# yoyololicon/pytorch-NMF

Hardware: AMD Instinct MI355X
Metric: MU GFLOP/s (algorithmic 8*N*C*R per iteration), dense NMF 4096x65536 rank-128 beta=1; MU iterations/s alongside (higher is better)
Workload: dtype f16; 1 GPU; NMF 4096x65536 rank=128 beta=1 (BASELINE configs[1]); preset=cfg1, rows=4096, cols_per_gpu=65536, rank=128, precision=f16, parallelism=single GPU, nsplit_h=16, nsplit_w=1, block_rows_h=256, block_rows_w=256, launch=eager launches

## Files before the change

### include/nmfmu.h

```cpp
#ifndef NMFMU_H_
#define NMFMU_H_

#include <stddef.h>
#include <stdint.h>

#ifdef __cplusplus
extern "C" {
#endif

#define NMFMU_ABI_VERSION 10

#define NMFMU_OK 0
#define NMFMU_ERR_UNSUPPORTED (-2)
#define NMFMU_ERR_ARG (-3)
#define NMFMU_ERR_ALLOC (-4)

#define NMFMU_PREC_BF16 0
#define NMFMU_PREC_BF16X3 1
#define NMFMU_PREC_F16 2
#define NMFMU_PREC_F16X 3
#define NMFMU_PREC_F16R 4

#define NMFMU_BETA_KL 0
#define NMFMU_BETA_EUC 1
#define NMFMU_BETA_IS 2
#define NMFMU_BETA_GEN 3

#define NMFMU_STAGE_REG 0
#define NMFMU_STAGE_DMA 1
#define NMFMU_STAGE_DMA_NOP2 3
#define NMFMU_STAGE_DMA_LDSTR 4
#define NMFMU_STAGE_DMA_SP128 5
#define NMFMU_STAGE_DMA_SPLIT 2

typedef struct nmfmu_factor {
  float* f;
  void* p1_hi;
  void* p1_lo;
  void* p2_hi;
  void* p2_lo;
  float* colsum;
  float* colsum_part;
  int32_t rows;
  int32_t rows_pad;
} nmfmu_factor;

typedef struct nmfmu_step {
  const void* xp;
  nmfmu_factor owner;
  nmfmu_factor panel;
  float* slab_num;
  float* slab_den;
  int32_t rank;
  int32_t r_pad;
  int32_t nsplit;
  int32_t precision;
  int32_t stage;
  int32_t block_rows;
  float beta;
  float gamma;
  float l1, l2;
  uint32_t* status;
  void* stamps;
} nmfmu_step;

// ... 334 lines not shown
```

### pytorch-nmf_amd/csrc/nmfmu_capi.hip

```cpp
#include <hip/hip_runtime.h>
#include <stdint.h>

#include <algorithm>
#include <cstdlib>
#include <new>
#include <vector>

#include "../../include/nmfmu.h"
#include "nmfmu_aux.h"
#include "nmfmu_fused.h"
#include "nmfmu_pp.h"
#include "nmfmu_sp.h"
#include "nmfmu_sp2.h"
#include "nmfmu_sp128.h"

#ifndef NMFMU_SP
#define NMFMU_SP 1
#endif
#ifndef NMFMU_SP2
#define NMFMU_SP2 1
#endif
#ifndef NMFMU_FUSE_APPLY_TWO_ACC
#define NMFMU_FUSE_APPLY_TWO_ACC 1
#endif
// ... 25 lines not shown
static bool pp_ldstr_eligible(int r_pad, int precision, float beta) {
  return pp_eligible(r_pad, precision, beta) && pp_trl_available(r_pad, is_f16(precision) ? kOpF16 : kOpBf16, kModeMU);
}
static bool sp128_eligible(int r_pad, int precision, float beta) {
  return pp_ldstr_eligible(r_pad, precision, beta) && precision == NMFMU_PREC_F16 && sp128_available(r_pad, kOpF16, kModeMU);
}
static bool sp_eligible(int r_pad, int precision, float beta) {
  return NMFMU_SP && nmfmu_beta_kind(beta) == NMFMU_BETA_KL && r_pad == 256 && precision == NMFMU_PREC_F16;
}
static bool sp2_eligible(int r_pad, int precision, float beta) {
  const int k = nmfmu_beta_kind(beta);
  return NMFMU_SP2 && (k == NMFMU_BETA_IS || k == NMFMU_BETA_GEN) && r_pad == 128 && precision == NMFMU_PREC_F16;
}
static int kernel_beta_kind(float beta) {
  if (beta == 0.5f) return kSqrt;
  if (beta == 1.5f) return kSqrt3;
  return nmfmu_beta_kind(beta);
}

struct GramRef {
  const float* gram;
  const void* hi;
  const void* lo;
  const float* scale;
};

int fused_dispatch(const nmfmu_step* st, int mode, float* loss_part, int M, int K, hipStream_t s,
                   const float* fuse_kl_den = nullptr, bool fuse_apply = false, const GramRef* gm = nullptr) {
  if (!st || !st->owner.p1_hi || !st->panel.p1_hi) return NMFMU_ERR_ARG;
  if (!st->xp && (mode == kModeMU || mode == kModeXB)) return NMFMU_ERR_ARG;
  if (st->owner.rows_pad % kRowPad || st->panel.rows_pad % kRowPad) return NMFMU_ERR_ARG;
  if (st->block_rows != 128 && st->block_rows != 256) return NMFMU_ERR_ARG;
  if (st->stage != NMFMU_STAGE_DMA && st->stage != NMFMU_STAGE_DMA_SPLIT && st->stage != NMFMU_STAGE_DMA_NOP2 &&
      st->stage != NMFMU_STAGE_DMA_LDSTR && st->stage != NMFMU_STAGE_DMA_SP128)
    return NMFMU_ERR_UNSUPPORTED;
  const bool sp128 = st->stage == NMFMU_STAGE_DMA_SP128;
  const bool ldstr = (st->stage == NMFMU_STAGE_DMA_LDSTR || sp128) && mode != kModeLoss;
  if (ldstr && (mode != kModeMU || st->block_rows != 256 || !pp_ldstr_eligible(st->r_pad, st->precision, st->beta)))
    return NMFMU_ERR_UNSUPPORTED;
  if (sp128 && !sp128_eligible(st->r_pad, st->precision, st->beta)) return NMFMU_ERR_UNSUPPORTED;
  if (st->stage == NMFMU_STAGE_DMA_SPLIT && mode == kModeMU && !(st->precision == NMFMU_PREC_BF16X3)) {
    if (nmfmu_beta_kind(st->beta) != NMFMU_BETA_KL || st->block_rows != 128) return NMFMU_ERR_UNSUPPORTED;
    mode = kModeMU2;
  }
  if (st->r_pad != pad_rank(st->rank) || st->nsplit < 1) return NMFMU_ERR_ARG;
  const bool x3 = st->precision == NMFMU_PREC_BF16X3;
  if (x3 && (!st->owner.p1_lo || !st->panel.p1_lo)) return NMFMU_ERR_ARG;
  const int kind = nmfmu_beta_kind(st->beta);
  if (st->precision == NMFMU_PREC_F16R && kind == NMFMU_BETA_EUC) return NMFMU_ERR_UNSUPPORTED;
  FusedArgs a{};
  a.xp = st->xp;
  a.p1_hi = static_cast<const uint16_t*>(st->panel.p1_hi);
  a.p1_lo = static_cast<const uint16_t*>(st->panel.p1_lo);
  a.p2_hi = static_cast<const uint16_t*>(st->panel.p2_hi);
  a.p2_lo = static_cast<const uint16_t*>(st->panel.p2_lo);
  a.a1_hi = static_cast<const uint16_t*>(st->owner.p1_hi);
  a.a1_lo = static_cast<const uint16_t*>(st->owner.p1_lo);
  a.slab_num = st->slab_num;
  a.slab_den = st->slab_den;
  a.loss_part = loss_part;
  a.M = M;
  a.K = K;
  a.M_pad = st->owner.rows_pad;
  a.ktiles = st->panel.rows_pad / kBK;
  a.nsplit = st->nsplit;
  a.tiles_per_split = (a.ktiles + st->nsplit - 1) / st->nsplit;
  a.beta = st->beta;
  a.status = st->status;
  a.cs_owner = st->owner.colsum;
// ... 9 lines not shown
    a.l1 = st->l1, a.l2 = st->l2, a.gamma = st->gamma;
  }
  if (mode == kModeMU2) {
    if (!a.slab_num || !a.p2_hi || fuse_apply) return NMFMU_ERR_ARG;
  } else if (mode == kModeXB) {
    if (kind != kEuc || x3 || st->block_rows != 128) return NMFMU_ERR_UNSUPPORTED;
    if (!a.p2_hi || (!fuse_apply && !a.slab_num)) return NMFMU_ERR_ARG;
    if (fuse_apply && (!gm || st->r_pad > 128)) return NMFMU_ERR_ARG;
    if (gm) {
      if (!gm->hi || !gm->lo || !gm->scale || (!fuse_apply && !a.slab_den)) return NMFMU_ERR_ARG;
      a.gram_hi = static_cast<const uint16_t*>(gm->hi), a.gram_lo = static_cast<const uint16_t*>(gm->lo);
      a.gram_scale = gm->scale;
    } else {
      a.slab_den = nullptr;
    }
  } else if (mode == kModeMU || mode == kModeDen) {
    if (!a.slab_num || !a.p2_hi || (x3 && !a.p2_lo)) return NMFMU_ERR_ARG;
    if (mode == kModeMU && kind != kKL && !a.slab_den) return NMFMU_ERR_ARG;
    if (mode == kModeDen && (kind != kGen || st->block_rows != 128)) return NMFMU_ERR_UNSUPPORTED;
  } else if (!loss_part) {
    return NMFMU_ERR_ARG;
  }
  const int grid = (st->owner.rows_pad / st->block_rows) * st->nsplit;
  if (st->block_rows == 256) {
    if (!st->xp || mode == kModeDen || !pp_eligible(st->r_pad, st->precision, st->beta)) return NMFMU_ERR_UNSUPPORTED;
    a.tiles_per_split = (a.tiles_per_split + 1) & ~1;
    a.debug = mode == kModeMU ? st->stamps : nullptr;
#ifdef NMFMU_DEBUG_HOOKS
    if (mode == kModeMU && g_pp_debug) a.debug = g_pp_debug;
#endif
    if (ldstr) a.o2_hi = nullptr;
    if (sp128 && mode == kModeMU && !loss_part) {
      a.tiles_per_split = (a.tiles_per_split + 3) & ~3;
      return launch_sp128(st->r_pad, kOpF16, a, grid, s);
    }
    return launch_pp(st->r_pad, is_f16(st->precision) ? kOpF16 : kOpBf16, mode, a, grid, s, st->precision == NMFMU_PREC_F16R,
                      mode == kModeMU && loss_part != nullptr, ldstr);
  }
  if (mode == kModeMU && sp_eligible(st->r_pad, st->precision, st->beta)) {
    a.tiles_per_split = (a.tiles_per_split + 3) & ~3;
    a.debug = st->stamps;
#ifdef NMFMU_DEBUG_HOOKS
    if (g_pp_debug) a.debug = g_pp_debug;
#endif
    if (st->stage == NMFMU_STAGE_DMA_NOP2) a.o2_hi = nullptr;
    return launch_sp(st->r_pad, kOpF16, a, grid, s);
  }
  if (mode == kModeMU && sp2_eligible(st->r_pad, st->precision, st->beta)) {
    a.tiles_per_split = (a.tiles_per_split + 3) & ~3;
    return launch_sp2(st->r_pad, kernel_beta_kind(st->beta), a, grid, s);
  }
  const int kk = kernel_beta_kind(st->beta);
#ifdef NMFMU_DEBUG_HOOKS
  a.debug = mode == kModeXB ? g_pp_debug : nullptr;
#endif
  switch (st->r_pad) {
    case 32: return launch_fused_r32(kk, st->precision, mode, a, grid, s);
    case 64: return launch_fused_r64(kk, st->precision, mode, a, grid, s);
    case 128: return launch_fused_r128(kk, st->precision, mode, a, grid, s);
    case 256: return launch_fused_r256(kk, st->precision, mode, a, grid, s);
  }
  return NMFMU_ERR_UNSUPPORTED;
}

struct Timer {
  std::vector<hipEvent_t> ev;
};
// ... 168 lines not shown
  const int64_t plane = (int64_t)st->owner.rows_pad * st->r_pad;
  int e = launch_slab_reduce(st->slab_num, st->nsplit, plane, num_out, S(stream));
  if (e) return e;
  if (den_out) {
    if (!st->slab_den) return NMFMU_ERR_ARG;
    e = launch_slab_reduce(st->slab_den, st->nsplit, plane, den_out, S(stream));
  }
  return e;
}

static int apply_common(const nmfmu_step* st, const float* num, const float* den, int nslab, const float* kl_den,
                        int trainer, float ortho, float* grad, void* stream, int den_nslab = 0, int skip_colsum = 0) {
  if (!st || !st->owner.f) return NMFMU_ERR_ARG;
  const bool kl = nmfmu_beta_kind(st->beta) == NMFMU_BETA_KL;
  ApplyArgs a{};
  a.f = st->owner.f;
  a.num = num ? num : st->slab_num;
  a.den = num ? den : st->slab_den;
  a.nslab = num ? nslab : st->nsplit;
  a.kl_den = kl ? kl_den : nullptr;
  if (!a.num || a.nslab < 1) return NMFMU_ERR_ARG;
  a.den_nslab = den_nslab;
  a.skip_colsum = skip_colsum;
  if (kl ? !a.kl_den : !a.den) return NMFMU_ERR_ARG;
  a.p1_hi = st->owner.p1_hi, a.p1_lo = st->owner.p1_lo, a.p2_hi = st->owner.p2_hi, a.p2_lo = st->owner.p2_lo;
  a.colsum_part = st->owner.colsum_part, a.colsum = st->owner.colsum;
  a.rows = st->owner.rows, a.rank = st->rank, a.rows_pad = st->owner.rows_pad;
  a.l1 = st->l1, a.l2 = st->l2, a.gamma = st->gamma;
  a.trainer = trainer, a.ortho = ortho, a.grad = grad;
  a.f16 = is_f16(st->precision);
  a.status = st->status;
  if (!a.p1_hi || !a.p2_hi || !a.colsum || !a.colsum_part) return NMFMU_ERR_ARG;
  if (st->stage == NMFMU_STAGE_DMA_NOP2 && sp_eligible(st->r_pad, st->precision, st->beta)) a.p2_hi = a.p2_lo = nullptr;
  if (st->stage == NMFMU_STAGE_DMA_LDSTR || st->stage == NMFMU_STAGE_DMA_SP128) {
    if (st->block_rows != 256 || !pp_ldstr_eligible(st->r_pad, st->precision, st->beta)) return NMFMU_ERR_UNSUPPORTED;
    a.p2_hi = a.p2_lo = nullptr;
  }
  return launch_apply(st->r_pad, a, st->precision == NMFMU_PREC_BF16X3, false, S(stream));
}

int nmfmu_mu_apply(const nmfmu_step* st, const float* num, const float* den, int nslab, const float* kl_den,
                   void* stream) {
  return apply_common(st, num, den, nslab, kl_den, 0, 0.f, nullptr, stream);
}

int nmfmu_trainer_apply(const nmfmu_step* st, const float* num, const float* den, int nslab, const float* kl_den,
                        float ortho, float* grad, void* stream) {
  if (!(ortho >= 0.f)) return NMFMU_ERR_ARG;
  return apply_common(st, num, den, nslab, kl_den, 1, ortho, grad, stream);
}

int nmfmu_xb_supported(int r_pad, int precision, float beta) {
  if (nmfmu_beta_kind(beta) != NMFMU_BETA_EUC) return 0;
  if (r_pad != 32 && r_pad != 64 && r_pad != 128 && r_pad != 256) return 0;
  if (precision == NMFMU_PREC_F16X) return r_pad <= 128;
  return precision == NMFMU_PREC_BF16 || precision == NMFMU_PREC_F16;
}

int nmfmu_xb_partial(const nmfmu_step* st, void* stream) {
  if (!st) return NMFMU_ERR_ARG;
  if (!nmfmu_xb_supported(st->r_pad, st->precision, st->beta)) return NMFMU_ERR_UNSUPPORTED;
  return fused_dispatch(st, kModeXB, nullptr, st->owner.rows, st->panel.rows, S(stream));
}

int nmfmu_xb_step(const nmfmu_step* st, const void* g_hi, const void* g_lo, const float* g_scale, int phase, void* stream) {
  if (!st || !g_hi || !g_lo || !g_scale || phase < 0 || phase > 2) return NMFMU_ERR_ARG;
  if (!nmfmu_xb_supported(st->r_pad, st->precision, st->beta)) return NMFMU_ERR_UNSUPPORTED;
// ... 248 lines not shown
```

### pytorch-nmf_amd/csrc/nmfmu_inst_sp128.hip

```cpp
#include "nmfmu_sp128.h"

namespace nmfmu {

bool sp128_available(int r_pad, int opt, int mode) { return r_pad == 128 && opt == kOpF16 && mode == kModeMU; }

int launch_sp128(int r_pad, int opt, const FusedArgs& a, int grid, hipStream_t s) {
  if (r_pad == 128 && opt == kOpF16) return launch_sp128_one<kOpF16>(a, grid, s);
  return -2;
}

}
```

### pytorch-nmf_amd/csrc/nmfmu_sp128.h

```cpp
#pragma once
#include "nmfmu_sp.h"

namespace nmfmu {

template <int OPT>
struct SP128Cfg {
  static constexpr int R_PAD = 128;
  static constexpr int BM = 256, WAVES = 4, THREADS = 256;
  static constexpr int KS = R_PAD / 16, RT = R_PAD / 32, ROWB = 2 * R_PAD, IMG = kBK * ROWB;
  static constexpr int NSLOT = 4, PF = 4;
  static constexpr int N1 = 2 * KS, N2 = 4 * RT;
  static constexpr int NPW = IMG / 1024 / WAVES;
  static constexpr int XTILE = BM * kBK * 2;
  static constexpr int GOPS = 10;
  static constexpr int NEL = 16 * GOPS;
  static constexpr int LDS_MAIN = NSLOT * IMG;
  static constexpr int LDS_EPI = 2 * WAVES * 32 * R_PAD * 4;
  static constexpr int LDS_BYTES = LDS_MAIN > LDS_EPI ? LDS_MAIN : LDS_EPI;
  static_assert(OPT == kOpF16, "fp16 operands");
  static_assert(N1 == 16 && N2 == 16 && NPW == 4 && NSLOT * IMG <= 65536, "schedule tables below; every LDS offset an immediate");
};

template <int OPT>
__global__ void __launch_bounds__(256, 1) sp128_kernel(const FusedArgs a) {
  using C = SP128Cfg<OPT>;
  constexpr int R_PAD = C::R_PAD, KS = C::KS, RT = C::RT, ROWB = C::ROWB, IMG = C::IMG, PF = C::PF, N1 = C::N1, N2 = C::N2;
  using u32x2 = __attribute__((ext_vector_type(2))) uint32_t;
  extern __shared__ __attribute__((aligned(16))) char smem[];

  const int tid = threadIdx.x;
  const int lane = tid & 63;
  const int wave = __builtin_amdgcn_readfirstlane(tid >> 6);
  const int j = lane & 31;
  const int hl = lane >> 5;
  const int mb = blockIdx.x / a.nsplit;
  const int ks = blockIdx.x - mb * a.nsplit;
  const int t0 = ks * a.tiles_per_split;
  const int t1 = min(t0 + a.tiles_per_split, a.ktiles);
  const int nt = t1 - t0;

  asm volatile("s_setreg_imm32_b32 hwreg(HW_REG_MODE, 23, 1), 1");
  auto stamp = [&](int slot) {
    unsigned long long* dbg = reinterpret_cast<unsigned long long*>(a.debug);
    if (!dbg || wave != 0) return;
    const unsigned long long c = __builtin_amdgcn_s_memtime();
    const unsigned long long r = __builtin_amdgcn_s_memrealtime();
    if (lane == 0) {
      if (blockIdx.x == 0) {
        dbg[slot * 4 + 0] = c;
        dbg[slot * 4 + 1] = r;
        dbg[slot * 4 + 2] = (unsigned long long)(nt > 0 ? nt : 0);
      }
      dbg[64 + 5 * blockIdx.x + slot] = r;
      if (slot == 2)
        dbg[64 + 5 * blockIdx.x + 4] = ((unsigned long long)__builtin_amdgcn_s_getreg(20 | (31 << 11)) << 32) |
                                       (unsigned long long)__builtin_amdgcn_s_getreg(4 | (31 << 11));
    }
  };
// ... 79 lines not shown
    auto load_x1 = [&](const char* src, u32x4(&x)[4], auto qc) {
      constexpr int qi = decltype(qc)::value;
      const unsigned l16 = lane16;
      u32x4& dst = x[qi];
      asm volatile("global_load_dwordx4 %0, %1, %2 offset:%3 nt" : "=&v"(dst) : "v"(l16), "s"(src), "n"(qi * 1024) : "memory");
    };
    auto wait_x = [&](auto cntc, u32x4(&x)[2][4]) {
      asm volatile("s_waitcnt vmcnt(%8)"
                   : "+v"(x[0][0]), "+v"(x[0][1]), "+v"(x[0][2]), "+v"(x[0][3]), "+v"(x[1][0]), "+v"(x[1][1]), "+v"(x[1][2]), "+v"(x[1][3])
                   : "n"(decltype(cntc)::value)
                   : "memory");
    };
    auto barrier = [&]() { asm volatile("s_barrier" ::: "memory"); };
    auto ratio_op = [&](auto kc, auto sbc) {
      constexpr int k = decltype(kc)::value, sb = decltype(sbc)::value, GO = C::GOPS;
      constexpr int g = k / GO, pos = k % GO, og = g >> 3, tt = (g >> 2) & 1, d = 2 * (g & 3);
      if constexpr (pos < 4) {
        float& r = er[pos];
        const float sv = S[sb][og][tt][2 * d + pos];
        asm volatile("v_rcp_f32 %0, %1" : "=v"(r) : "v"(sv));
      } else if constexpr (pos < 8) {
        constexpr int p = pos - 4;
        float& r = er[p];
        const uint32_t w = xb[sb][og][2 * tt + (d >> 2)][(d & 3) + (p >> 1)];
        if constexpr ((p & 1) == 0) asm volatile("v_fma_mix_f32 %0, %1, %0, 0 op_sel_hi:[1,0,0]" : "+v"(r) : "v"(w));
        else asm volatile("v_fma_mix_f32 %0, %1, %0, 0 op_sel:[1,0,0] op_sel_hi:[1,0,0]" : "+v"(r) : "v"(w));
      } else {
        constexpr int h = pos - 8;
        uint32_t& g2 = gn[og][tt][d + h];
        const float e0 = er[2 * h], e1 = er[2 * h + 1];
        asm volatile("v_cvt_pk_f16_f32 %0, %1, %2" : "=v"(g2) : "v"(e0), "v"(e1));
      }
    };
    auto issue_g1 = [&](auto kc, auto slotc, auto rsc) {
      constexpr int k = decltype(kc)::value, tt = k & 1, kk = k >> 1, rs = decltype(rsc)::value;
      u32x4& dst = r128[rs];
      const int ad = ga[kk];
      asm volatile("ds_read_b128 %0, %1 offset:%2" : "=v"(dst) : "v"(ad), "n"(tt * 16 * ROWB + decltype(slotc)::value * IMG));
    };
    auto issue_g2 = [&](auto kc, auto slotc, auto rsc) {
      constexpr int k = decltype(kc)::value, rt = k % RT, c4 = k / RT, tt = c4 >> 1, m2 = c4 & 1, rs = decltype(rsc)::value;
      constexpr int o0 = (16 * tt + 8 * m2) * ROWB + decltype(slotc)::value * IMG;
      u32x2 &dlo = rlo[rs], &dhi = rhi[rs];
      const int a0 = gb[2 * m2][rt], a1 = gb[2 * m2 + 1][rt];
      asm volatile("ds_read_b64_tr_b16 %0, %1 offset:%2" : "=v"(dlo) : "v"(a0), "n"(o0));
      asm volatile("ds_read_b64_tr_b16 %0, %1 offset:%2" : "=v"(dhi) : "v"(a1), "n"(o0 + 4 * ROWB));
    };
    auto mfma_g1 = [&](auto kc, auto nbc, auto rsc, auto ogc) {
      constexpr int k = decltype(kc)::value, tt = k & 1, kk = k >> 1, nb = decltype(nbc)::value, rs = decltype(rsc)::value;
      constexpr int og = decltype(ogc)::value;
      f32x16& sd = S[nb][og][tt];
      const u32x4 pa = r128[rs], qo = q[og][kk];
      const f32x16 seed = epsv;
      if constexpr (kk == 0) asm volatile("v_mfma_f32_32x32x16_f16 %0, %1, %2, %3" : "=&v"(sd) : "v"(pa), "a"(qo), "v"(seed));
      else asm volatile("v_mfma_f32_32x32x16_f16 %0, %1, %2, %0" : "+v"(sd) : "v"(pa), "a"(qo));
    };
    auto mfma_g2 = [&](auto kc, auto rsc, auto ogc) {
      constexpr int k = decltype(kc)::value, rt = k % RT, c4 = k / RT, tt = c4 >> 1, m2 = c4 & 1, rs = decltype(rsc)::value;
      constexpr int og = decltype(ogc)::value;
      const u32x4 nh = {gn[og][tt][4 * m2], gn[og][tt][4 * m2 + 1], gn[og][tt][4 * m2 + 2], gn[og][tt][4 * m2 + 3]};
      const u32x4 bh = {rlo[rs][0], rlo[rs][1], rhi[rs][0], rhi[rs][1]};
      f32x16& ad = acc[og][rt];
      asm volatile("v_mfma_f32_32x32x16_f16 %0, %1, %2, %0" : "+a"(ad) : "v"(nh), "v"(bh));
    };
    auto issue_entry = [&](auto nc, auto lastc) {
      constexpr int n = decltype(nc)::value;
      constexpr SPEnt e = sp_entry<N1, N2>(n, decltype(lastc)::value);
      using RS = std::integral_constant<int, n % PF>;
      if constexpr (e.g1) issue_g1(std::integral_constant<int, e.k>{}, std::integral_constant<int, (e.it + 1) & 3>{}, RS{});
      else issue_g2(std::integral_constant<int, e.k>{}, std::integral_constant<int, e.it & 3>{}, RS{});
    };
    auto ratio_gap = [&](auto gapc, auto sbc) {
      constexpr int gi = decltype(gapc)::value, per = C::NEL / 32;
      static_assert(C::NEL % 32 == 0, "whole instructions per gap");
      static_for<per>([&](auto cc) { ratio_op(std::integral_constant<int, gi * per + decltype(cc)::value>{}, sbc); });
    };

    auto group = [&](int i0, auto lastc) {
      constexpr bool last = decltype(lastc)::value;
      constexpr int LEN = sp_group_len<N1, N2>(last);
      const char* dsrc = nullptr;
      const char* xs0 = nullptr;
      const char* xs1 = nullptr;
      static_for<PF>([&](auto pc) { issue_entry(pc, lastc); });
      static_for<LEN>([&](auto nc) {
        constexpr int n = decltype(nc)::value;
        constexpr SPEnt e = sp_entry<N1, N2>(n, last);
        constexpr bool final_it = last && e.it == 3;
        using RS = std::integral_constant<int, n % PF>;
        using K = std::integral_constant<int, e.k>;
        using SB = std::integral_constant<int, e.it & 1>;
        using OG0 = std::integral_constant<int, 0>;
        using OG1 = std::integral_constant<int, 1>;
        if constexpr (final_it && e.k == 0)
          static_for<C::NEL>([&](auto kc) { ratio_op(kc, SB{}); });
        asm volatile("s_waitcnt lgkmcnt(%0)" ::"n"(sp_younger<N1, N2, PF>(n, last)));
        if constexpr (e.g1) {
          using NB = std::integral_constant<int, (e.it + 1) & 1>;
          mfma_g1(K{}, NB{}, RS{}, OG0{});
          if constexpr (e.k == 0) {
            dsrc = panel_src(i0 + e.it + 3);
            xs0 = x_src(i0 + e.it + 2, 0);
            xs1 = x_src(i0 + e.it + 2, 1);
          }
          ratio_gap(std::integral_constant<int, 2 * e.k>{}, SB{});
          mfma_g1(K{}, NB{}, RS{}, OG1{});
          if constexpr (n + PF < LEN) issue_entry(std::integral_constant<int, n + PF>{}, lastc);
          ratio_gap(std::integral_constant<int, 2 * e.k + 1>{}, SB{});
          if constexpr (e.k == N1 - 1) {
            asm volatile("s_waitcnt vmcnt(8)" ::: "memory");
            barrier();
          }
        } else {
          mfma_g2(K{}, RS{}, OG0{});
          if constexpr (!final_it) {
            if constexpr (e.k < C::NPW) dma_piece(dsrc, K{}, std::integral_constant<int, (e.it + 3) & 3>{});
            if constexpr (e.k >= 8 && e.k < 12) load_x1(xs0, xb[e.it & 1][0], std::integral_constant<int, e.k - 8>{});
            if constexpr (e.k >= 12) load_x1(xs1, xb[e.it & 1][1], std::integral_constant<int, e.k - 12>{});
          }
          mfma_g2(K{}, RS{}, OG1{});
          if constexpr (n + PF < LEN) issue_entry(std::integral_constant<int, n + PF>{}, lastc);
          if constexpr (!final_it && e.k == N2 - 1) {
            wait_x(std::integral_constant<int, 12>{}, xb[(e.it + 1) & 1]);
          }
        }
      });
    };

    {
      static_for<3>([&](auto tc) {
        const char* src = panel_src(decltype(tc)::value);
        asm volatile("s_nop 4" ::: "memory");
        static_for<C::NPW>([&](auto pc) { dma_piece(src, pc, tc); });
      });
      const char* x00 = x_src(0, 0);
      const char* x01 = x_src(0, 1);
      const char* x10 = x_src(1, 0);
      const char* x11 = x_src(1, 1);
      asm volatile("s_nop 4" ::: "memory");
      static_for<4>([&](auto qc) { load_x1(x00, xb[0][0], qc); });
      static_for<4>([&](auto qc) { load_x1(x01, xb[0][1], qc); });
      static_for<4>([&](auto qc) { load_x1(x10, xb[1][0], qc); });
      static_for<4>([&](auto qc) { load_x1(x11, xb[1][1], qc); });
      wait_x(std::integral_constant<int, 0>{}, xb[0]);
      wait_x(std::integral_constant<int, 0>{}, xb[1]);
      static_for<2 * KS>([&](auto kc) {
        u32x4& r = q[decltype(kc)::value / KS][decltype(kc)::value % KS];
        asm volatile("" : "+a"(r));
      });
      barrier();
      using Z = std::integral_constant<int, 0>;
      static_for<PF>([&](auto pc) { issue_g1(pc, Z{}, pc); });
      static_for<N1>([&](auto kc) {
        constexpr int k = decltype(kc)::value;
        constexpr int younger = (N1 - 1 - k) < (PF - 1) ? (N1 - 1 - k) : (PF - 1);
        asm volatile("s_waitcnt lgkmcnt(%0)" ::"n"(younger));
        mfma_g1(kc, Z{}, std::integral_constant<int, k % PF>{}, Z{});
        mfma_g1(kc, Z{}, std::integral_constant<int, k % PF>{}, std::integral_constant<int, 1>{});
        if constexpr (k + PF < N1) issue_g1(std::integral_constant<int, k + PF>{}, Z{}, std::integral_constant<int, k % PF>{});
      });
      asm volatile("s_nop 15\n\ts_nop 7" ::: "memory");
    }
    stamp(0);
    int i0 = 0;
    for (; i0 + 4 < nt; i0 += 4) group(i0, std::false_type{});
    group(i0, std::true_type{});
    stamp(1);
    asm volatile("s_nop 15\n\ts_nop 15" ::: "memory");
    wait_x(std::integral_constant<int, 0>{}, xb[0]);
    wait_x(std::integral_constant<int, 0>{}, xb[1]);
  }
  __syncthreads();

  int tid_e = tid;
  asm volatile("" : "+v"(tid_e));
  const int lane_e = tid_e & 63, j_e = lane_e & 31, hl_e = lane_e >> 5;
  if (a.fuse_apply) {
    constexpr int LDT = R_PAD;
    constexpr int SP = R_PAD / 8;
    constexpr int NCH = (32 * SP) / 64;
    const int slot_e = lane_e % SP, rl0 = lane_e / SP;
    float den8[8];
#pragma unroll
    for (int k = 0; k < 8; ++k) den8[k] = a.kl_den[slot_e * 8 + k];
    const bool vec = (a.rank & 3) == 0;
    bool clamped = false;
    static_for<2 * RT>([&](auto rc) {
      constexpr int og = decltype(rc)::value / RT, rt = decltype(rc)::value % RT;
      float* tile = reinterpret_cast<float*>(smem) + (2 * wave + og) * (32 * LDT);
#pragma unroll
      for (int e = 0; e < 16; ++e) tile[((e & 3) + 8 * (e >> 2) + 4 * hl_e) * LDT + rt * 32 + j_e] = acc[og][rt][e];
    });
    __syncthreads();
    const bool plain = a.l1 <= 0.f && a.l2 <= 0.f && a.gamma == 1.f && a.rank == R_PAD && mb * C::BM + C::BM <= a.M;
    float csum8[2][8], rden8[8];
#pragma unroll
    for (int k = 0; k < 8; ++k) rden8[k] = 1.f / den8[k];
#pragma unroll
    for (int og = 0; og < 2; ++og) {
// ... 104 lines not shown
    }
    __syncthreads();
    float* red = reinterpret_cast<float*>(smem);
#pragma unroll
    for (int og = 0; og < 2; ++og)
#pragma unroll
      for (int k = 0; k < 8; ++k) {
        float tot = csum8[og][k];
        tot += __shfl_xor(tot, 32, 64);
        tot += __shfl_xor(tot, 16, 64);
        if (lane_e < SP) red[(2 * wave + og) * R_PAD + slot_e * 8 + k] = tot;
      }
    __syncthreads();
    for (int r = tid_e; r < R_PAD; r += C::THREADS) {
      float tot = (red[r] + red[R_PAD + r]) + (red[2 * R_PAD + r] + red[3 * R_PAD + r]);
      tot += (red[4 * R_PAD + r] + red[5 * R_PAD + r]) + (red[6 * R_PAD + r] + red[7 * R_PAD + r]);
      a.colsum_part[(size_t)mb * R_PAD + r] = tot;
    }
  } else {
    static_for<2 * RT>([&](auto rc) {
      constexpr int og = decltype(rc)::value / RT, rt = decltype(rc)::value % RT;
      const size_t slab = ((size_t)ks * a.M_pad + (size_t)(mb * C::BM + (2 * wave + og) * 32)) * R_PAD;
#pragma unroll
      for (int e = 0; e < 16; ++e) {
        const int row = (e & 3) + 8 * (e >> 2) + 4 * hl_e;
        a.slab_num[slab + (size_t)row * R_PAD + rt * 32 + j_e] = acc[og][rt][e];
      }
    });
  }
  if (a.debug) asm volatile("s_waitcnt vmcnt(0)" ::: "memory");
  stamp(3);
}

template <int OPT>
int launch_sp128_one(const FusedArgs& a, int grid, hipStream_t s) {
  using C = SP128Cfg<OPT>;
  return launch_with_dynamic_lds<sp128_kernel<OPT>, C::THREADS, C::LDS_BYTES>(dim3(grid), s, a);
}

int launch_sp128(int r_pad, int opt, const FusedArgs& a, int grid, hipStream_t s);
bool sp128_available(int r_pad, int opt, int mode);

}
```

### pytorch-nmf_amd/torchnmf_amd/_capi.py

```python
from __future__ import annotations

import ctypes as C
import os
from typing import Optional

LIB_NAME = 'libnmfmu.so'
LIB_PATH = os.environ.get('NMFMU_LIB') or os.path.join(os.path.dirname(os.path.abspath(__file__)), LIB_NAME)

OK = 0
ERR_UNSUPPORTED = -2
ERR_ARG = -3
ERR_ALLOC = -4
PREC_BF16, PREC_BF16X3, PREC_F16, PREC_F16X, PREC_F16R = 0, 1, 2, 3, 4
STAGE_REG, STAGE_DMA, STAGE_DMA_SPLIT = 0, 1, 2
STAGE_DMA_NOP2 = 3
STAGE_DMA_LDSTR = 4
STAGE_DMA_SP128 = 5
BETA_KL, BETA_EUC, BETA_IS, BETA_GEN = 0, 1, 2, 3
KERNEL_FUSED, KERNEL_PP, KERNEL_SP = 0, 1, 2

PRECISIONS = {'bf16': PREC_BF16, 'bf16x3': PREC_BF16X3, 'f16': PREC_F16, 'f16x': PREC_F16X, 'f16r': PREC_F16R}


class NmfmuError(RuntimeError):
    pass


class Factor(C.Structure):
    _fields_ = [('f', C.c_void_p), ('p1_hi', C.c_void_p), ('p1_lo', C.c_void_p), ('p2_hi', C.c_void_p),
                ('p2_lo', C.c_void_p), ('colsum', C.c_void_p), ('colsum_part', C.c_void_p), ('rows', C.c_int32),
                ('rows_pad', C.c_int32)]


class Step(C.Structure):
    _fields_ = [('xp', C.c_void_p), ('owner', Factor), ('panel', Factor), ('slab_num', C.c_void_p),
                ('slab_den', C.c_void_p), ('rank', C.c_int32), ('r_pad', C.c_int32), ('nsplit', C.c_int32),
                ('precision', C.c_int32), ('stage', C.c_int32), ('block_rows', C.c_int32), ('beta', C.c_float), ('gamma', C.c_float),
                ('l1', C.c_float), ('l2', C.c_float), ('status', C.c_void_p), ('stamps', C.c_void_p)]


class GemmDesc(C.Structure):
    _fields_ = [('a_hi', C.c_void_p), ('a_lo', C.c_void_p), ('b_hi', C.c_void_p), ('b_lo', C.c_void_p),
                ('m_pad', C.c_int32), ('n_pad', C.c_int32), ('k_pad', C.c_int32), ('precision', C.c_int32),
                ('beta', C.c_float), ('x', C.c_void_p), ('gn_hi', C.c_void_p), ('gn_lo', C.c_void_p),
                ('gp_hi', C.c_void_p), ('gp_lo', C.c_void_p), ('out', C.c_void_p), ('m_valid', C.c_int32),
                ('n_valid', C.c_int32), ('ops', C.c_int32), ('t_batch', C.c_int32), ('t_rank', C.c_int32),
                ('t_taps', C.c_int32), ('t_lh', C.c_int32), ('tile_rows', C.c_int32), ('n_ld', C.c_int32), ('k_len', C.c_int32), ('k_split', C.c_int32),
                ('tail_rows', C.c_int32), ('rag_c0', C.c_int32), ('rag_channels', C.c_int32),
                ('win_nd', C.c_int32), ('win_lh', C.c_int32 * 3), ('win_taps', C.c_int32 * 3), ('win_channels', C.c_int32),
                ('win_pitch', C.c_int32), ('win_fold', C.c_int32), ('t_koff', C.c_void_p), ('stage_mode', C.c_int32)]
# ... 258 lines not shown
```

### pytorch-nmf_amd/torchnmf_amd/engine.py

```python
from __future__ import annotations

import ctypes as C
import os
from typing import Optional

import torch

from . import _capi


def _ptr(t: Optional[torch.Tensor]) -> Optional[int]:
    return None if t is None else t.data_ptr()


class HipBackend:

    name = 'hip'

    def __init__(self):
        self.lib = _capi.load()
        if not torch.cuda.is_available():
            raise _capi.NmfmuError('torchnmf_amd needs a ROCm device (MI355X); none is visible and there is no '
                                   'CPU fallback')

# ... 456 lines not shown
        gamma = mu_gamma(self.beta)
        dev = V.device

        self.fW = FactorBuf(W, self.r_pad, self.precision, self.be)
        self.fH = FactorBuf(H, self.r_pad, self.precision, self.be)
        self.flags = torch.tensor([0, 0x7f800000], dtype=torch.int32, device=dev)
        self.status = torch.zeros(1, dtype=torch.int32, device=dev)
        n_pad, c_pad = self.fH.rows_pad, self.fW.rows_pad
        def tile_rows(m_pad, k_pad):
            if block_rows is not None:
                return block_rows
            if hasattr(self.be, 'step_block_rows'):
                return self.be.step_block_rows(m_pad, k_pad, self.r_pad, self.precision, self.beta, dev)
            return self.be.block_rows(self.r_pad, self.precision, self.beta)
        br = tile_rows(n_pad, c_pad)
        self.block_rows = br
        xp_h = self.be.pack_x(V, False, self.precision, br, n_pad, c_pad, self.flags)
        ns_h = self._nsplit(n_pad, c_pad, br, dev)
        need_den = False if self.kl else ('one' if self.gram_path else True)
        self.step_h = StepBuf(xp_h, self.fH, self.fW, R, self.r_pad, ns_h, self.precision, stage, br, self.beta, gamma,
                              l1, l2, need_den=need_den, status=self.status)
        self.step_w = None
        if update_W:
            brw = tile_rows(c_pad, n_pad)
            xp_w = self.be.pack_x(V, True, self.precision, brw, c_pad, n_pad, None)
            ns_w = self._nsplit(c_pad, n_pad, brw, dev)
            self.step_w = StepBuf(xp_w, self.fW, self.fH, R, self.r_pad, ns_w, self.precision, stage, brw, self.beta,
                                  gamma, l1, l2, need_den=need_den, status=self.status)
        if sp128_auto and dev.type == 'cuda':
            ncu = torch.cuda.get_device_properties(dev).multi_processor_count
            steps = (self.step_h, self.step_w)
            if all(st.block_rows == 256 and (st.owner.rows_pad // 256) * st.nsplit >= ncu
                   and (st.panel.rows_pad // 64) % (4 * st.nsplit) == 0 for st in steps):
                for st in steps:
                    st.struct.stage = _capi.STAGE_DMA_SP128
        self.gm = self.be.gram_alloc(self.r_pad, dev) if self.gram_path else None
        self.timer: Optional[KernelTimer] = None
        self.refresh_images()
        self.loss_part = torch.empty(max((n_pad // br) * ns_h, 1), dtype=torch.float32, device=dev)
        self.loss_out = torch.zeros(1, dtype=torch.float64, device=dev)
        self._riding = None
        self._riding_pending = False
        if (group is None and self.kl and self.step_w is not None and update_H and hasattr(self.be, 'riding_supported')
                and os.environ.get('TORCHNMF_AMD_RIDING_LOSS', '1') != '0' and V.dtype == torch.float32 and V.stride(1) == 1
                and self.be.riding_supported(self.step_w)):
            self._riding = {'V': V, 'bufs': None}
        if group is not None:
            tail = self.r_pad if self.kl else self.step_h.plane
            self.xbuf = torch.empty(self.step_h.plane + tail, dtype=torch.float32, device=dev)
            explicit_direct = bool(ar_direct)
            if ar_direct is None:
                ar_direct = os.environ.get('TORCHNMF_AMD_COMM', 'torch') == 'c'
            self._comm = None
            if ar_direct and hasattr(self.be, 'comm_init'):
                self._comm = self.be.comm_init(group, dev)
                ar_overlap = False
            elif explicit_direct:
                raise _capi.NmfmuError("allreduce='direct' needs the library's own RCCL communicator (nmfmu_comm_*), which "
                                       f"the {getattr(self.be, 'name', type(self.be).__name__)} backend does not provide")
            st = self.step_h
            nblk = st.owner.rows_pad // 256
            frac = float(os.environ.get('TORCHNMF_AMD_AR_SPLIT', '0.5'))
            r0 = min(max(int(frac * nblk + 1e-9), 1), max(nblk - 1, 1)) * 256
            self._h_rows = None
            if ar_overlap is None:
                ar_overlap = os.environ.get('TORCHNMF_AMD_AR_OVERLAP', '0') != '0'
            if (ar_overlap and nblk >= 2 and st.owner.rows > r0
                    and hasattr(self.be, 'xp_rows')):
# ... 197 lines not shown
```

Baseline: 925,800 GFLOP/s.

## Spread SP128 ratio reciprocals into MFMA gaps via compile-time schedule tables

Splits the per-element ratio work in the SP128 kernel into separate reciprocal, multiply and pack steps, and moves RB=48 reciprocals into the first-GEMM phase, interleaved between MFMAs. Compile-time tables place the remaining multiplies and packs with a minimum distance from their producers. The aim is to hide the transcendental/VALU ratio cost behind matrix-core work instead of bunching it at the phase boundary. It adds register pressure and schedule complexity, and keeps the old behaviour behind an RB0 stage and environment switch.

```diff
diff --git a/include/nmfmu.h b/include/nmfmu.h
--- a/include/nmfmu.h
+++ b/include/nmfmu.h
@@ -31,6 +31,7 @@
 #define NMFMU_STAGE_DMA_NOP2 3
 #define NMFMU_STAGE_DMA_LDSTR 4
 #define NMFMU_STAGE_DMA_SP128 5
+#define NMFMU_STAGE_DMA_SP128_RB0 6
 #define NMFMU_STAGE_DMA_SPLIT 2
 
 typedef struct nmfmu_factor {
diff --git a/pytorch-nmf_amd/csrc/nmfmu_capi.hip b/pytorch-nmf_amd/csrc/nmfmu_capi.hip
--- a/pytorch-nmf_amd/csrc/nmfmu_capi.hip
+++ b/pytorch-nmf_amd/csrc/nmfmu_capi.hip
@@ -81,9 +81,10 @@
   if (st->owner.rows_pad % kRowPad || st->panel.rows_pad % kRowPad) return NMFMU_ERR_ARG;
   if (st->block_rows != 128 && st->block_rows != 256) return NMFMU_ERR_ARG;
   if (st->stage != NMFMU_STAGE_DMA && st->stage != NMFMU_STAGE_DMA_SPLIT && st->stage != NMFMU_STAGE_DMA_NOP2 &&
-      st->stage != NMFMU_STAGE_DMA_LDSTR && st->stage != NMFMU_STAGE_DMA_SP128)
+      st->stage != NMFMU_STAGE_DMA_LDSTR && st->stage != NMFMU_STAGE_DMA_SP128 && st->stage != NMFMU_STAGE_DMA_SP128_RB0)
     return NMFMU_ERR_UNSUPPORTED;
-  const bool sp128 = st->stage == NMFMU_STAGE_DMA_SP128;
+  const bool sp128_rb0 = st->stage == NMFMU_STAGE_DMA_SP128_RB0;
+  const bool sp128 = st->stage == NMFMU_STAGE_DMA_SP128 || sp128_rb0;
   const bool ldstr = (st->stage == NMFMU_STAGE_DMA_LDSTR || sp128) && mode != kModeLoss;
   if (ldstr && (mode != kModeMU || st->block_rows != 256 || !pp_ldstr_eligible(st->r_pad, st->precision, st->beta)))
     return NMFMU_ERR_UNSUPPORTED;
@@ -159,7 +160,7 @@
     if (ldstr) a.o2_hi = nullptr;
     if (sp128 && mode == kModeMU && !loss_part) {
       a.tiles_per_split = (a.tiles_per_split + 3) & ~3;
-      return launch_sp128(st->r_pad, kOpF16, a, grid, s);
+      return sp128_rb0 ? launch_sp128_rb0(st->r_pad, kOpF16, a, grid, s) : launch_sp128(st->r_pad, kOpF16, a, grid, s);
     }
     return launch_pp(st->r_pad, is_f16(st->precision) ? kOpF16 : kOpBf16, mode, a, grid, s, st->precision == NMFMU_PREC_F16R,
                       mode == kModeMU && loss_part != nullptr, ldstr);
@@ -394,7 +395,7 @@
   a.status = st->status;
   if (!a.p1_hi || !a.p2_hi || !a.colsum || !a.colsum_part) return NMFMU_ERR_ARG;
   if (st->stage == NMFMU_STAGE_DMA_NOP2 && sp_eligible(st->r_pad, st->precision, st->beta)) a.p2_hi = a.p2_lo = nullptr;
-  if (st->stage == NMFMU_STAGE_DMA_LDSTR || st->stage == NMFMU_STAGE_DMA_SP128) {
+  if (st->stage == NMFMU_STAGE_DMA_LDSTR || st->stage == NMFMU_STAGE_DMA_SP128 || st->stage == NMFMU_STAGE_DMA_SP128_RB0) {
     if (st->block_rows != 256 || !pp_ldstr_eligible(st->r_pad, st->precision, st->beta)) return NMFMU_ERR_UNSUPPORTED;
     a.p2_hi = a.p2_lo = nullptr;
   }
diff --git a/pytorch-nmf_amd/csrc/nmfmu_inst_sp128.hip b/pytorch-nmf_amd/csrc/nmfmu_inst_sp128.hip
--- a/pytorch-nmf_amd/csrc/nmfmu_inst_sp128.hip
+++ b/pytorch-nmf_amd/csrc/nmfmu_inst_sp128.hip
@@ -1,11 +1,15 @@
 #include "nmfmu_sp128.h"
+
+#ifndef NMFMU_SP128_RB
+#define NMFMU_SP128_RB 48
+#endif
 
 namespace nmfmu {
 
 bool sp128_available(int r_pad, int opt, int mode) { return r_pad == 128 && opt == kOpF16 && mode == kModeMU; }
 
 int launch_sp128(int r_pad, int opt, const FusedArgs& a, int grid, hipStream_t s) {
-  if (r_pad == 128 && opt == kOpF16) return launch_sp128_one<kOpF16>(a, grid, s);
+  if (r_pad == 128 && opt == kOpF16) return launch_sp128_one<kOpF16, NMFMU_SP128_RB>(a, grid, s);
   return -2;
 }
 
diff --git a/pytorch-nmf_amd/csrc/nmfmu_inst_sp128_rb0.hip b/pytorch-nmf_amd/csrc/nmfmu_inst_sp128_rb0.hip
--- /dev/null
+++ b/pytorch-nmf_amd/csrc/nmfmu_inst_sp128_rb0.hip
@@ -0,0 +1,10 @@
+#include "nmfmu_sp128.h"
+
+namespace nmfmu {
+
+int launch_sp128_rb0(int r_pad, int opt, const FusedArgs& a, int grid, hipStream_t s) {
+  if (r_pad == 128 && opt == kOpF16) return launch_sp128_one<kOpF16, 0>(a, grid, s);
+  return -2;
+}
+
+}
diff --git a/pytorch-nmf_amd/csrc/nmfmu_sp128.h b/pytorch-nmf_amd/csrc/nmfmu_sp128.h
--- a/pytorch-nmf_amd/csrc/nmfmu_sp128.h
+++ b/pytorch-nmf_amd/csrc/nmfmu_sp128.h
@@ -21,9 +21,66 @@
   static_assert(N1 == 16 && N2 == 16 && NPW == 4 && NSLOT * IMG <= 65536, "schedule tables below; every LDS offset an immediate");
 };
 
-template <int OPT>
+constexpr int kSP128Dist = 24;
+constexpr bool sp128_b_busy(int gap) { return (gap & 1) == 0 && ((gap >> 1) < 4 || (gap >> 1) >= 8); }
+struct SP128PhaseB {
+  int first[33];
+};
+constexpr SP128PhaseB sp128_phase_b(int rb) {
+  int cnt[32] = {};
+  int left = rb;
+  for (int pass = 0; pass < 7; ++pass)
+    for (int g = 3; g < 32; ++g) {
+      const int cls = (g & 1) ? 0 : sp128_b_busy(g) ? 2 : 1;
+      if (left > 0 && cls == (pass == 6 ? 0 : pass >> 1)) ++cnt[g], --left;
+    }
+  SP128PhaseB t{};
+  for (int g = 0; g < 32; ++g) t.first[g + 1] = t.first[g] + cnt[g];
+  return t;
+}
+struct SP128PhaseA {
+  int first[33];
+  int op[160];
+};
+constexpr SP128PhaseA sp128_phase_a(int rb) {
+  SP128PhaseA t{};
+  int pos_r[64] = {}, pos_m[64] = {};
+  for (int x = 0; x < 64; ++x) pos_r[x] = -1000;
+  int nr = rb, nm = 0, nc = 0, pos = 0;
+  int cost_left = 2 * (64 - rb) + 64 + 32;
+  for (int g = 0; g < 32; ++g) {
+    t.first[g] = pos;
+    const bool flush = g == 31;
+    const int budget = (cost_left + (32 - g) - 1) / (32 - g);
+    int used = 0;
+    for (int c = 0; c < 2 && nr < 64 && used + 2 <= budget; ++c) {
+      pos_r[nr] = pos;
+      t.op[pos++] = nr++;
+      used += 2;
+    }
+    while (nm < 64 && nm < nr && (flush || (used < budget && pos - pos_r[nm] >= kSP128Dist))) {
+      pos_m[nm] = pos;
+      t.op[pos++] = 64 + nm++;
+      ++used;
+    }
+    while (nc < 32 && 2 * nc + 1 < nm && (flush || (used < budget && pos - pos_m[2 * nc + 1] >= kSP128Dist))) {
+      t.op[pos++] = 128 + nc++;
+      ++used;
+    }
+    cost_left -= used;
+  }
+  t.first[32] = pos;
+  return t;
+}
+template <int RB>
+inline constexpr SP128PhaseA kSP128TabA = sp128_phase_a(RB);
+template <int RB>
+inline constexpr SP128PhaseB kSP128TabB = sp128_phase_b(RB);
+
+template <int OPT, int RB>
 __global__ void __launch_bounds__(256, 1) sp128_kernel(const FusedArgs a) {
   using C = SP128Cfg<OPT>;
+  static_assert(RB >= 0 && RB <= 64 && RB % 16 == 0, "whole S tiles' worth of units");
   constexpr int R_PAD = C::R_PAD, KS = C::KS, RT = C::RT, ROWB = C::ROWB, IMG = C::IMG, PF = C::PF, N1 = C::N1, N2 = C::N2;
   using u32x2 = __attribute__((ext_vector_type(2))) uint32_t;
   extern __shared__ __attribute__((aligned(16))) char smem[];
@@ -169,6 +226,40 @@
         asm volatile("v_cvt_pk_f16_f32 %0, %1, %2" : "=v"(g2) : "v"(e0), "v"(e1));
       }
     };
+    auto rcp_x = [&](auto xc, auto sbc) {
+      constexpr int x = decltype(xc)::value, sb = decltype(sbc)::value, u = x >> 2, pos = x & 3;
+      constexpr int tt = u >> 3, og = (u >> 2) & 1, d = 2 * (u & 3);
+      float r = S[sb][og][tt][2 * d + pos];
+      asm volatile("v_rcp_f32 %0, %0" : "+v"(r));
+      S[sb][og][tt][2 * d + pos] = r;
+    };
+    auto mul_x = [&](auto xc, auto sbc) {
+      constexpr int x = decltype(xc)::value, sb = decltype(sbc)::value, u = x >> 2, p = x & 3;
+      constexpr int tt = u >> 3, og = (u >> 2) & 1, d = 2 * (u & 3);
+      float r = S[sb][og][tt][2 * d + p];
+      const uint32_t w = xb[sb][og][2 * tt + (d >> 2)][(d & 3) + (p >> 1)];
+      if constexpr ((p & 1) == 0) asm volatile("v_fma_mix_f32 %0, %1, %0, 0 op_sel_hi:[1,0,0]" : "+v"(r) : "v"(w));
+      else asm volatile("v_fma_mix_f32 %0, %1, %0, 0 op_sel:[1,0,0] op_sel_hi:[1,0,0]" : "+v"(r) : "v"(w));
+      S[sb][og][tt][2 * d + p] = r;
+    };
+    auto pack_y = [&](auto yc, auto sbc) {
+      constexpr int y = decltype(yc)::value, sb = decltype(sbc)::value, u = y >> 1, h = y & 1;
+      constexpr int tt = u >> 3, og = (u >> 2) & 1, d = 2 * (u & 3);
+      uint32_t& g2 = gn[og][tt][d + h];
+      const float e0 = S[sb][og][tt][2 * d + 2 * h], e1 = S[sb][og][tt][2 * d + 2 * h + 1];
+      asm volatile("v_cvt_pk_f16_f32 %0, %1, %2" : "=v"(g2) : "v"(e0), "v"(e1));
+    };
+    auto table_op = [&](auto cc, auto sbc) {
+      constexpr int code = kSP128TabA<RB>.op[decltype(cc)::value], kind = code >> 6;
+      using I = std::integral_constant<int, code & 63>;
+      if constexpr (kind == 0) rcp_x(I{}, sbc);
+      else if constexpr (kind == 1) mul_x(I{}, sbc);
+      else pack_y(I{}, sbc);
+    };
+    auto rcp_gap = [&](auto gapc, auto sbc) {
+      constexpr int gi = decltype(gapc)::value, lo = kSP128TabB<RB>.first[gi], n = kSP128TabB<RB>.first[gi + 1] - lo;
+      static_for<n>([&](auto cc) { rcp_x(std::integral_constant<int, lo + decltype(cc)::value>{}, sbc); });
+    };
     auto issue_g1 = [&](auto kc, auto slotc, auto rsc) {
       constexpr int k = decltype(kc)::value, tt = k & 1, kk = k >> 1, rs = decltype(rsc)::value;
       u32x4& dst = r128[rs];
@@ -210,8 +301,25 @@
     auto ratio_gap = [&](auto gapc, auto sbc) {
       constexpr int gi = decltype(gapc)::value, per = C::NEL / 32;
       static_assert(C::NEL % 32 == 0, "whole instructions per gap");
-      static_for<per>([&](auto cc) { ratio_op(std::integral_constant<int, gi * per + decltype(cc)::value>{}, sbc); });
-    };
+      if constexpr (RB == 0) {
+        static_for<per>([&](auto cc) { ratio_op(std::integral_constant<int, gi * per + decltype(cc)::value>{}, sbc); });
+      } else {
+        constexpr int lo = kSP128TabA<RB>.first[gi], n = kSP128TabA<RB>.first[gi + 1] - lo;
+        static_for<n>([&](auto cc) { table_op(std::integral_constant<int, lo + decltype(cc)::value>{}, sbc); });
+      }
+    };
+#ifdef NMFMU_SP128_PHASE_STAMPS
+    unsigned long long ph_sum[2] = {0, 0}, ph_last = __builtin_amdgcn_s_memtime();
+    auto phase_end = [&](int which) {
+      const unsigned long long c = __builtin_amdgcn_s_memtime();
+      ph_sum[which] += c - ph_last;
+      ph_last = c;
+    };
+    auto phase_reset = [&]() { ph_last = __builtin_amdgcn_s_memtime(); };
+#else
+    auto phase_end = [&](int) {};
+    auto phase_reset = [&]() {};
+#endif
 
     auto group = [&](int i0, auto lastc) {
       constexpr bool last = decltype(lastc)::value;
@@ -230,12 +338,21 @@
         using OG0 = std::integral_constant<int, 0>;
         using OG1 = std::integral_constant<int, 1>;
         if constexpr (final_it && e.k == 0)
-          static_for<C::NEL>([&](auto kc) { ratio_op(kc, SB{}); });
+          static_for<C::NEL - RB>([&](auto kc) {
+            if constexpr (RB == 0) ratio_op(kc, SB{});
+            else table_op(kc, SB{});
+          });
+        if constexpr (e.k == 0) phase_end(e.g1 || final_it ? 1 : 0);
+        if constexpr (RB > 0 && e.g1 && e.k == 0) {
+          dsrc = panel_src(i0 + e.it + 3);
+          xs0 = x_src(i0 + e.it + 2, 0);
+          xs1 = x_src(i0 + e.it + 2, 1);
+        }
         asm volatile("s_waitcnt lgkmcnt(%0)" ::"n"(sp_younger<N1, N2, PF>(n, last)));
         if constexpr (e.g1) {
           using NB = std::integral_constant<int, (e.it + 1) & 1>;
           mfma_g1(K{}, NB{}, RS{}, OG0{});
-          if constexpr (e.k == 0) {
+          if constexpr (RB == 0 && e.k == 0) {
             dsrc = panel_src(i0 + e.it + 3);
             xs0 = x_src(i0 + e.it + 2, 0);
             xs1 = x_src(i0 + e.it + 2, 1);
@@ -254,9 +371,12 @@
             if constexpr (e.k < C::NPW) dma_piece(dsrc, K{}, std::integral_constant<int, (e.it + 3) & 3>{});
             if constexpr (e.k >= 8 && e.k < 12) load_x1(xs0, xb[e.it & 1][0], std::integral_constant<int, e.k - 8>{});
             if constexpr (e.k >= 12) load_x1(xs1, xb[e.it & 1][1], std::integral_constant<int, e.k - 12>{});
+            if constexpr (RB > 0) rcp_gap(std::integral_constant<int, 2 * e.k>{}, std::integral_constant<int, (e.it + 1) & 1>{});
           }
           mfma_g2(K{}, RS{}, OG1{});
           if constexpr (n + PF < LEN) issue_entry(std::integral_constant<int, n + PF>{}, lastc);
+          if constexpr (RB > 0 && !final_it)
+            rcp_gap(std::integral_constant<int, 2 * e.k + 1>{}, std::integral_constant<int, (e.it + 1) & 1>{});
           if constexpr (!final_it && e.k == N2 - 1) {
             wait_x(std::integral_constant<int, 12>{}, xb[(e.it + 1) & 1]);
           }
@@ -297,11 +417,20 @@
         if constexpr (k + PF < N1) issue_g1(std::integral_constant<int, k + PF>{}, Z{}, std::integral_constant<int, k % PF>{});
       });
       asm volatile("s_nop 15\n\ts_nop 7" ::: "memory");
+      static_for<RB>([&](auto xc) { rcp_x(xc, Z{}); });
     }
     stamp(0);
+    phase_reset();
     int i0 = 0;
     for (; i0 + 4 < nt; i0 += 4) group(i0, std::false_type{});
     group(i0, std::true_type{});
+    phase_end(1);
+#ifdef NMFMU_SP128_PHASE_STAMPS
+    if (a.debug && wave == 0 && blockIdx.x == 0 && lane == 0) {
+      unsigned long long* dbg = reinterpret_cast<unsigned long long*>(a.debug);
+      dbg[16] = ph_sum[0], dbg[17] = ph_sum[1], dbg[18] = (unsigned long long)nt;
+    }
+#endif
     stamp(1);
     asm volatile("s_nop 15\n\ts_nop 15" ::: "memory");
     wait_x(std::integral_constant<int, 0>{}, xb[0]);
@@ -472,13 +601,14 @@
   stamp(3);
 }
 
-template <int OPT>
+template <int OPT, int RB>
 int launch_sp128_one(const FusedArgs& a, int grid, hipStream_t s) {
   using C = SP128Cfg<OPT>;
-  return launch_with_dynamic_lds<sp128_kernel<OPT>, C::THREADS, C::LDS_BYTES>(dim3(grid), s, a);
+  return launch_with_dynamic_lds<sp128_kernel<OPT, RB>, C::THREADS, C::LDS_BYTES>(dim3(grid), s, a);
 }
 
 int launch_sp128(int r_pad, int opt, const FusedArgs& a, int grid, hipStream_t s);
+int launch_sp128_rb0(int r_pad, int opt, const FusedArgs& a, int grid, hipStream_t s);
 bool sp128_available(int r_pad, int opt, int mode);
 
 }
diff --git a/pytorch-nmf_amd/torchnmf_amd/_capi.py b/pytorch-nmf_amd/torchnmf_amd/_capi.py
--- a/pytorch-nmf_amd/torchnmf_amd/_capi.py
+++ b/pytorch-nmf_amd/torchnmf_amd/_capi.py
@@ -16,6 +16,7 @@
 STAGE_DMA_NOP2 = 3
 STAGE_DMA_LDSTR = 4
 STAGE_DMA_SP128 = 5
+STAGE_DMA_SP128_RB0 = 6
 BETA_KL, BETA_EUC, BETA_IS, BETA_GEN = 0, 1, 2, 3
 KERNEL_FUSED, KERNEL_PP, KERNEL_SP = 0, 1, 2
 
diff --git a/pytorch-nmf_amd/torchnmf_amd/engine.py b/pytorch-nmf_amd/torchnmf_amd/engine.py
--- a/pytorch-nmf_amd/torchnmf_amd/engine.py
+++ b/pytorch-nmf_amd/torchnmf_amd/engine.py
@@ -512,8 +512,9 @@
             steps = (self.step_h, self.step_w)
             if all(st.block_rows == 256 and (st.owner.rows_pad // 256) * st.nsplit >= ncu
                    and (st.panel.rows_pad // 64) % (4 * st.nsplit) == 0 for st in steps):
+                rb0 = os.environ.get('TORCHNMF_AMD_SP128', '1') == 'rb0'
                 for st in steps:
-                    st.struct.stage = _capi.STAGE_DMA_SP128
+                    st.struct.stage = _capi.STAGE_DMA_SP128_RB0 if rb0 else _capi.STAGE_DMA_SP128
         self.gm = self.be.gram_alloc(self.r_pad, dev) if self.gram_path else None
         self.timer: Optional[KernelTimer] = None
         self.refresh_images()
```

New measurement: 948,700 GFLOP/s, median of 6. 1.02x the previous value.
